# sebproell/4C

Measured on AMD Instinct MI355X. Metric: element-evaluations/sec (hex8 linear elasticity, K+r global assembly), higher is better.
Workload: dtype f64; 1 GPU; hex8-linear-100^3-per-gpu; elements_global=1000000, elements_evaluated_per_gpu=1000000, dofs_owned_rank0=3090903, nnz_rank0=245438109

## Files before the change

4c_amd/csrc/fcg_context.cpp:

```cpp
#include <hip/hip_runtime.h>

#include <algorithm>
#include <chrono>
#include <climits>
#include <cstdlib>
#include <cstring>
#include <mutex>
#include <string>
#include <thread>
#include <vector>

#include "fcg_internal.hpp"
#include "fcg_status.hpp"
#include "fcg_shape.hpp"

namespace {

namespace plan = fcg::create;

std::mutex g_err_mutex;
std::string g_create_error;

void set_create_error(const std::string& s)
{
// ... 214 lines not shown
  U.up<int32_t>(&m.err, nullptr, 3);
  if (U.he == hipSuccess) U.he = hipHostMalloc(reinterpret_cast<void**>(&m.err_host), 2 * sizeof(int32_t),
      hipHostMallocDefault);
}

void upload_structured(Uploader& U, const fcg_desc* d, const plan::NodeRows& N, const plan::StructHost& sp)
{
  fcg::DeviceMesh& m = U.ctx->mesh;
  m.path = FCG_PATH_STRUCTURED;
  m.tiles_x = sp.tiles_x;
  m.tiles_y = sp.tiles_y;
  m.tiles_z = sp.tiles_z;
  m.seg_planes = sp.seg;
  m.I0 = sp.lo[0]; m.J0 = sp.lo[1]; m.K0 = sp.lo[2];
  m.NI = sp.n[0]; m.NJ = sp.n[1]; m.NK = sp.n[2];
  m.EX0 = sp.elo[0]; m.EY0 = sp.elo[1]; m.EZ0 = sp.elo[2];
  m.EX = sp.en[0]; m.EY = sp.en[1]; m.EZ = sp.en[2];
  const char* de = std::getenv("FCG_SWEEP_DEFER");
  m.sweep_defer = de && de[0] ? de[0] == '1'
                              : d->kinematics == FCG_LINEAR && 8 * sp.rows_unordered > N.nrn();
  U.up(&m.elem_at, sp.elem_at);
  U.up(&m.lat_x, sp.lat_x);
  U.up(&m.lat_dof, sp.lat_dof);
  U.up(&m.plane_rec, sp.plane_rec);
  std::vector<double> tab(8 * 8 * 3 * 2 + 8 + 24);
  double xi[81], w[27], xn[81];
  fcg::gauss_rule(fcg::kHex8, xi, w);
  fcg::node_param_coords(fcg::kHex8, xn);
  for (int g = 0; g < 8; ++g) fcg::shape_deriv(fcg::kHex8, &xi[3 * g], &tab[24 * g]);
  for (int g = 0; g < 8; ++g) fcg::shape_deriv(fcg::kHex8, &xn[3 * g], &tab[192 + 24 * g]);
  for (int g = 0; g < 8; ++g) tab[384 + g] = w[g];
  for (int k = 0; k < 24; ++k) tab[392 + k] = xi[k];
  U.up(&m.tables, tab);
}

void upload_colored(Uploader& U, const fcg_desc* d, const plan::Incidences& I, const plan::ColorHost& cp)
{
  fcg::DeviceMesh& m = U.ctx->mesh;
  m.path = FCG_PATH_COLORED;
  U.up(&m.inc_of, I.inc_of);
  U.up(&m.inc_pos, I.inc_pos);
  U.up(&m.inc_row0, I.inc_row0);
  m.h27_pencil = d->material == FCG_MAT_STVK;
  if (m.h27_pencil)
  {
    fcg::upload_h27_tables();
    U.up(&m.col_ele, cp.pen_ele.data(), d->n_ele);
    U.up(&m.pen_ptr, cp.pen_ptr);
    U.up(&m.ele_nb, cp.nb.data(), d->n_ele);
    for (int c = 0; c < 5; ++c) m.pen_color[c] = cp.pen_color[c];
  }
  else
  {
    U.up(&m.col_ele, cp.col_ele.data(), d->n_ele);
    U.up(&m.ele_ft, cp.ft.data(), d->n_ele);
    for (int c = 0; c < 9; ++c) m.color_ptr[c] = cp.color_ptr[c];
  }
}

void upload_gather(Uploader& U, const fcg_desc* d, const plan::GatherHost& G)
{
  fcg::DeviceMesh& m = U.ctx->mesh;
  m.path = FCG_PATH_GATHER;
  m.n_rec = G.n_rec;
  m.n_rec_single = G.n_single;
  m.n_multi = int64_t(G.multi_ptr.size()) - 1;
// ... 479 lines not shown
  }
  return FCG_OK;
}

int fcg_evaluate(fcg_ctx* ctx, int action, const double* u_col, double* fint_row, double* K_vals,
    int32_t* bad_ele_gid)
{
  return fcg_evaluate_host(ctx, action, FCG_ACCUMULATE, u_col, fint_row, K_vals, bad_ele_gid);
}

int fcg_set_timing(fcg_ctx* ctx, int enable)
{
  if (!ctx) return FCG_ERR_ARG;
  ctx->timing.enabled = enable != 0;
  return FCG_OK;
}

int fcg_get_timing(const fcg_ctx* ctx, double* ms_element, double* ms_assemble)
{
  if (!ctx) return FCG_ERR_ARG;
  read_timing(const_cast<fcg_ctx*>(ctx)->timing);
  if (ms_element) *ms_element = ctx->timing.ms_element;
  if (ms_assemble) *ms_assemble = ctx->timing.ms_assemble;
  return 2;
}

int fcg_get_diagnostics(const fcg_ctx* ctx, uint64_t* out, int n)
{
  if (!ctx || !out || n < 0) return FCG_ERR_ARG;
  const fcg::DeviceMesh& m = ctx->mesh;
  unsigned long long v[16] = {};
  if (m.stamps && hipMemcpy(v, m.stamps, sizeof(v), hipMemcpyDeviceToHost) != hipSuccess)
    return fcg_device_error();
  for (int i = 0; i < n && i < 16; ++i) out[i] = v[i];
  return m.stamps ? 16 : 0;
}

int fcg_get_create_phases(const fcg_ctx* ctx, double* out, int n)
{
  if (!ctx || (!out && n > 0)) return FCG_ERR_ARG;
  for (int i = 0; i < n && i < 8; ++i) out[i] = ctx->create_phase_s[i];
  return 8;
}

int fcg_get_info(const fcg_ctx* ctx, fcg_info* info)
{
  if (!ctx || !info) return FCG_ERR_ARG;
  const fcg::DeviceMesh& m = ctx->mesh;
  info->n_ele = m.n_ele;
  info->n_node = m.n_node;
  info->n_rows = m.n_rows;
  info->n_cols = m.n_cols;
  info->nnz = m.nnz;
  info->n_incidences = m.n_inc;
  info->scratch_bytes = !m.scratch ? 0
                                   : (m.h27_nslab > 1 ? m.h27_ring : m.n_inc) *
                                         fcg::record_doubles(m.npe) * int64_t(sizeof(double));
  info->device_bytes = ctx->device_bytes;
  info->path = m.path;
  info->h27_slabs =
      m.path == FCG_PATH_GENERAL && m.h27s ? int32_t(std::max<int64_t>(1, m.h27_nslab)) : 0;
  return FCG_OK;
}

int fcg_set_element_materials(fcg_ctx* ctx, int32_t n_mat, const double* youngs,
    const double* poisson, const int32_t* ele_mat)
// ... 126 lines not shown
```

4c_amd/csrc/fcg_internal.hpp:

```cpp
#pragma once

#include <hip/hip_runtime.h>

#include <cstdint>
#include <string>
#include <vector>

#include "fcg_create_plan.hpp"
#include "fourc_gpu.h"

namespace fcg {

#ifndef FCG_REC27
#define FCG_REC27 256
#endif
constexpr int64_t record_doubles(int npe) { return npe == 27 ? int64_t(FCG_REC27) : 9 * int64_t(npe) + 3; }

struct DeviceMesh {
  int celltype = 0, kinem = 0, npe = 8;
  int64_t n_ele = 0, n_node = 0, n_rows = 0, n_cols = 0, nnz = 0;
  int64_t n_rownodes = 0, n_inc = 0;
  double lambda = 0, mu = 0, cdiag = 0;
  int material = FCG_MAT_STVK;
  double nh_c = 0, nh_beta = 0;
// ... 28 lines not shown
  int64_t* multi_ptr = nullptr;
  int32_t* rec_row0 = nullptr;
  int32_t* rec_meta = nullptr;
  int64_t* rec_base = nullptr;
  int32_t* rec_ele = nullptr;
  uint8_t* rec_a = nullptr;
  uint32_t* rec_tmap = nullptr;
  bool h27s = false;
  int32_t* inc_ele = nullptr;
  uint8_t* inc_a = nullptr;
  int32_t* asm_order = nullptr;
  int32_t* ele_orig = nullptr;
  double* ele_x = nullptr;
  double* ele_gp = nullptr;
  int32_t gp_bad_code = 0, gp_bad_ele = 0;
  int32_t* ele_dof = nullptr;
  double* gather_dummy = nullptr;
  double* apply_ye = nullptr;
  int32_t* apply_dof = nullptr;
  double* diag_de = nullptr;
  uint8_t* diag_dbc = nullptr;
  int64_t h27_nslab = 0, h27_slab = 0, h27_ring = 0;
  int h27_el_grid = 512;
  std::vector<int64_t> h27_asm_ptr;
  int32_t* h27_rows = nullptr;
  int32_t* h27_rslot0 = nullptr;
  int32_t* h27_slot = nullptr;

  int path = FCG_PATH_GENERAL;
  int32_t tiles_x = 0, tiles_y = 0, tiles_z = 0, seg_planes = 0;
  int32_t I0 = 0, J0 = 0, K0 = 0, NI = 0, NJ = 0, NK = 0;
  int32_t EX0 = 0, EY0 = 0, EZ0 = 0, EX = 0, EY = 0, EZ = 0;
  bool sweep_defer = false;
  int32_t* elem_at = nullptr;
  double* lat_x = nullptr;
  int32_t* lat_dof = nullptr;
  uint32_t* plane_rec = nullptr;
  double* tables = nullptr;
  unsigned long long* stamps = nullptr;

  int32_t* col_lid = nullptr;
  int64_t* diag_pos = nullptr;
  bool square_local = false;
  bool owned_cols_first = false;
  bool triple_rows = true;
  double* pcg_work = nullptr;
  int64_t pcg_n = 0;

  int32_t* node_dof_row = nullptr;
  int32_t* node_dof_kcol = nullptr;
  int64_t* mass_ptr = nullptr;
  int64_t* mass_inc = nullptr;
  double* mass_tab = nullptr;
  double* mass_rho = nullptr;
  int32_t* mass_bad = nullptr;
};

hipError_t launch_sweep_h8(const DeviceMesh& m, const double* d_u_col, bool want_k,
    bool overwrite, double* d_K, double* d_fint, hipStream_t stream);

struct SweepTsi {
  const double* v_col = nullptr;
  const double* T_col = nullptr;
  const double* Ngp = nullptr;
  double* Kst = nullptr;
  double* Kts = nullptr;
  double* Ktt = nullptr;
  double* fT = nullptr;
  double m = 0, T0 = 0, conduct = 0, kts = 0;
  bool split = true;
};
hipError_t launch_sweep_h8_tsi(const DeviceMesh& m, const double* d_u_col, bool overwrite,
    double* d_K, double* d_fint, const SweepTsi& t, hipStream_t stream);

struct Timing {
  bool enabled = false;
  bool pending = false;
  int path = 0;
  bool fused = false;
  hipEvent_t ev[3] = {nullptr, nullptr, nullptr};
  double ms_element = 0.0, ms_assemble = 0.0;
};

struct HostStaging {
  double* pin[2] = {nullptr, nullptr};
  hipEvent_t ev[2] = {nullptr, nullptr};
  hipStream_t stream = nullptr;
  int64_t chunk = 0;
  int threads = 8;
};
hipError_t staged_copy(HostStaging& st, int device, void* dst, const void* src, int64_t bytes,
    bool to_device);
// ... 55 lines not shown
```

4c_amd/csrc/fcg_sweep.hip:

```cpp
#include <hip/hip_runtime.h>

#include "fcg_hex8_element.hpp"
#include "fcg_internal.hpp"
#include "fcg_visit_table.h"

namespace fcg {

namespace {

constexpr int TX = 4, TY = 4;
constexpr int EXN = TX + 1, EYN = TY + 1;
constexpr int NSLOT = EXN * EYN;
constexpr int NXN = TX + 2;
constexpr int NNODE = NXN * (TY + 2);
constexpr int PR_ROW0 = 0, PR_LEN = 16, PR_BASE = 32, PR_NPOS = 64;
__device__ constexpr int nx_sw(int p, int slot) { return (p + 4 * (slot & 1)) & 7; }
__device__ constexpr int nx2i(int d, int p, int slot, int n)
{
  return (((d * 4 + p) * NSLOT + slot) * 8 + (n ^ nx_sw(p, slot))) * 2;
}

__device__ constexpr int node_ox(int n) { return ((n & 3) == 1 || (n & 3) == 2) ? 1 : 0; }
__device__ constexpr int node_oy(int n) { return (n & 3) >= 2 ? 1 : 0; }
__device__ constexpr int node_oz(int n) { return n >> 2; }
// ... 48 lines not shown
#ifdef FCG_PROBE_WG3
  double hold[1][9][TSI ? (TH ? 9 : 18) : 9];
#else
#if defined(FCG_HOLD9)
  static constexpr int kHs = 9;
#else
  static constexpr int kHs = 10;
#endif
  alignas(16) double hold[TX * TY + (TSI ? 0 : 1)][9][TSI ? (TH ? 9 : 18) : kHs];
#endif
#ifdef FCG_HOLDLO9
  double hold_lo[DEFER ? TX * TY : 1][9][9];
#else
  alignas(16) double hold_lo[DEFER ? TX * TY : 1][9][10];
#endif
};

__device__ inline int ring(int p) { return (p % 3 + 3) % 3; }

constexpr int kDppXor1 = 0xB1;
constexpr int kDppXor2 = 0x4E;
constexpr int kDppHalfMirror = 0x141;
constexpr int kDppRowRor8 = 0x128;
template <int CTRL>
__device__ inline double dpp_f64(double v)
{
  const int lo = __builtin_amdgcn_mov_dpp(__double2loint(v), CTRL, 0xF, 0xF, false);
  const int hi = __builtin_amdgcn_mov_dpp(__double2hiint(v), CTRL, 0xF, 0xF, false);
  return __hiloint2double(hi, lo);
}

__device__ inline int node_at(int ox, int oy, int oz) { return 4 * oz + (oy ? (ox ? 2 : 3) : (ox ? 1 : 0)); }

template <int KIN, bool TSI, class SH>
__device__ inline void sweep_stage_a(SH& sh, const SweepArgs& A, int s, int g,
    int sx, int sy, int L, int e)
{
  constexpr int NC = node_comps<TSI>();
  const bool valid = e >= 0;
  const double* nd[8];
#pragma unroll
  for (int n = 0; n < 8; ++n)
    nd[n] = sh.node[ring(L + node_oz(n))][(sy + node_oy(n)) * NXN + sx + node_ox(n)];
  const H8dN dn = h8_dn_products(sh.gxi[g][0], sh.gxi[g][1], sh.gxi[g][2]);
  double J[9];
#pragma unroll
  for (int q = 0; q < 9; ++q) J[q] = 0.0;
#pragma unroll
  for (int n = 0; n < 8; ++n)
  {
    const double x0 = nd[n][0], x1 = nd[n][1], x2 = nd[n][2];
    double d0, d1, d2;
    h8_dn(dn, n, d0, d1, d2);
    J[0] += d0 * x0; J[1] += d1 * x0; J[2] += d2 * x0;
    J[3] += d0 * x1; J[4] += d1 * x1; J[5] += d2 * x1;
    J[6] += d0 * x2; J[7] += d1 * x2; J[8] += d2 * x2;
  }
  int bad = 0;
  {
    const int ox = node_ox(g), oy = node_oy(g), oz = node_oz(g);
    const double* zl = sh.node[ring(L)][0];
    const double* zh = sh.node[ring(L + 1)][0];
    const double* pz = oz ? zh : zl;
    const int cxy = (sy + oy) * NXN + sx + ox;
    const double* o = pz + NC * cxy;
    const double* ex_ = pz + NC * (cxy + (ox ? -1 : 1));
    const double* ey_ = pz + NC * (cxy + (oy ? -NXN : NXN));
    const double* ez_ = (oz ? zl : zh) + NC * cxy;
    const double sgx = ox ? 1.0 : -1.0, sgy = oy ? 1.0 : -1.0, sgz = oz ? 1.0 : -1.0;
    const double a0 = sgx * (o[0] - ex_[0]), a1 = sgx * (o[1] - ex_[1]), a2 = sgx * (o[2] - ex_[2]);
    const double b0 = sgy * (o[0] - ey_[0]), b1 = sgy * (o[1] - ey_[1]), b2 = sgy * (o[2] - ey_[2]);
    const double c0 = sgz * (o[0] - ez_[0]), c1 = sgz * (o[1] - ez_[1]), c2 = sgz * (o[2] - ez_[2]);
    const double detn = a0 * (b1 * c2 - b2 * c1) + b0 * (c1 * a2 - c2 * a1) + c0 * (a1 * b2 - a2 * b1);
    if (detn == 0.0) bad = 2;
    else if (!(detn > 0)) bad = 1;
  }
  const double det = h8_invert3x3(J);
  if (det == 0.0) bad = 2;
  else if (TSI && det < 1e-16 && bad == 0) bad = 1;
  const double fac = det * sh.w8[g];
  const double sq = valid ? sqrt(fabs(fac)) : 0.0;
  const double cf = fac < 0.0 ? -sq : sq;
  if (KIN == 0)
  {
#pragma unroll
    for (int q = 0; q < 9; ++q) J[q] *= sq;
  }
  const double ns = KIN == 0 ? 1.0 : sq;
  auto nxyz = [&](int n, double& n0, double& n1, double& n2) {
    double d0, d1, d2;
    h8_dn(dn, n, d0, d1, d2);
    n0 = J[0] * d0 + J[3] * d1 + J[6] * d2;
    n1 = J[1] * d0 + J[4] * d1 + J[7] * d2;
    n2 = J[2] * d0 + J[5] * d1 + J[8] * d2;
  };
  double E[6] = {0, 0, 0, 0, 0, 0};
  double F[9] = {0, 0, 0, 0, 0, 0, 0, 0, 0};
  double Tg = 0.0, trv = 0.0;
#pragma unroll
  for (int n = 0; n < 8; ++n)
  {
    double n0, n1, n2;
    nxyz(n, n0, n1, n2);
    if (TSI)
    {
      trv += n0 * nd[n][6] + n1 * nd[n][7] + n2 * nd[n][8];
      Tg += sh.Ng[TSI ? g : 0][n] * nd[n][9];
    }
    sh.nx[nx2i(0, g >> 1, s, n) + (g & 1)] = KIN == 0 ? n0 : ns * n0;
    sh.nx[nx2i(1, g >> 1, s, n) + (g & 1)] = KIN == 0 ? n1 : ns * n1;
    sh.nx[nx2i(2, g >> 1, s, n) + (g & 1)] = KIN == 0 ? n2 : ns * n2;
    if (KIN == 1)
    {
// ... 17 lines not shown
      for (int q = 0; q < 3; ++q)
        C[r + 3 * q] = F[3 * r] * F[3 * q] + F[3 * r + 1] * F[3 * q + 1] + F[3 * r + 2] * F[3 * q + 2];
    E[0] = 0.5 * (C[0] - 1.0);
    E[1] = 0.5 * (C[4] - 1.0);
    E[2] = 0.5 * (C[8] - 1.0);
    E[3] = C[3];
    E[4] = C[7];
    E[5] = C[2];
  }
  if (KIN == 1)
  {
    const StVK& m = A.mat;
    double S[6];
    S[0] = m.cdiag * E[0] + m.lambda * E[1] + m.lambda * E[2];
    S[1] = m.lambda * E[0] + m.cdiag * E[1] + m.lambda * E[2];
    S[2] = m.lambda * E[0] + m.lambda * E[1] + m.cdiag * E[2];
    S[3] = m.mu * E[3];
    S[4] = m.mu * E[4];
    S[5] = m.mu * E[5];
    double* P = sh.gp[KIN ? g : 0][KIN ? s : 0];
#pragma unroll
    for (int q = 0; q < 9; ++q) P[q] = F[q];
#pragma unroll
    for (int q = 0; q < 6; ++q) P[9 + q] = S[q];
    P[15] = cf;
  }
  if (TSI)
  {
    double* t = sh.tg[TSI ? g : 0][TSI ? s : 0];
    t[0] = cf;
    t[1] = Tg;
    t[2] = A.tsi_m * cf * trv;
  }
  if (valid && bad)
  {
    atomicMax(&A.err[0], bad);
    atomicMin(&A.err[1], e);
  }
  const unsigned long long neg = __ballot(valid && fac < 0.0);
  if (g == 0) sh.neg[s] = uint32_t((neg >> (threadIdx.x & 56)) & 0xFFull);

}

template <int KIN, bool NEG, bool TSI, bool TH = false, class SH>
__device__ inline void sweep_visit(const SH& sh, int slot, int a, int b1, int b2,
    uint32_t nm, double* acc1, double* acc2)
{
#ifndef FCG_TH_PAIRS
#define FCG_TH_PAIRS 1
#endif
  double2 nA[TH && FCG_TH_PAIRS ? 4 : 1], n1[TH && FCG_TH_PAIRS ? 4 : 1], n2[TH && FCG_TH_PAIRS ? 4 : 1];
  if constexpr (TH && FCG_TH_PAIRS)
  {
#pragma unroll
    for (int p = 0; p < 4; ++p)
    {
      nA[p] = *reinterpret_cast<const double2*>(&sh.NgT[a][2 * p]);
      n1[p] = *reinterpret_cast<const double2*>(&sh.NgT[b1][2 * p]);
      n2[p] = *reinterpret_cast<const double2*>(&sh.NgT[b2][2 * p]);
    }
  }
  auto gp_body = [&](int g, double a0, double a1, double a2, double p0, double p1, double p2,
                     double q0, double q1, double q2) {
    if (TH)
    {
      const double* t = sh.tg[g][slot];
#if FCG_TH_PAIRS
      const double2 t01 = *reinterpret_cast<const double2*>(t), t23 = *reinterpret_cast<const double2*>(t + 2);
      const double cf = t01.x, Tg = t01.y, qq = t23.x;
      const double Na = (g & 1) ? nA[g >> 1].y : nA[g >> 1].x, N1 = (g & 1) ? n1[g >> 1].y : n1[g >> 1].x,
                   N2 = (g & 1) ? n2[g >> 1].y : n2[g >> 1].x;
#else
      const double cf = t[0], Tg = t[1], qq = t[2];
      const double Na = sh.Ng[g][a], N1 = sh.Ng[g][b1], N2 = sh.Ng[g][b2];
// ... 136 lines not shown
__device__ inline void block_k(const StVK& m, const double* acc, double* Kb)
{
  const double lam = m.lambda, mu = m.mu;
#pragma unroll
  for (int r = 0; r < 3; ++r)
#pragma unroll
    for (int q = 0; q < 3; ++q) Kb[3 * r + q] = lam * acc[3 * r + q] + mu * acc[3 * q + r];
  if (KIN == 0)
  {
    const double tr = mu * (acc[0] + acc[4] + acc[8]);
    Kb[0] += tr;
    Kb[4] += tr;
    Kb[8] += tr;
  }
  else
  {
    Kb[0] += mu * acc[9] + acc[15];
    Kb[4] += mu * acc[10] + acc[15];
    Kb[8] += mu * acc[11] + acc[15];
    Kb[1] += mu * acc[12]; Kb[3] += mu * acc[12];
    Kb[5] += mu * acc[13]; Kb[7] += mu * acc[13];
    Kb[2] += mu * acc[14]; Kb[6] += mu * acc[14];
  }
}

#define FCG_STAMP(i)                                                                               \
  if (A.stamps && tid == 0)                                                                        \
  {                                                                                                \
    const unsigned long long now = __builtin_amdgcn_s_memtime();                                  \
    st_acc[i] += now - st_last;                                                                    \
    st_last = now;                                                                                 \
  }

template <int KIN, bool WANT_K, bool OVERWRITE, int MODE>
#ifndef FCG_SWEEP_WGS
#define FCG_SWEEP_WGS 2
#endif
__global__ __launch_bounds__(256, KIN ? 1 : FCG_SWEEP_WGS) void sweep_h8_kernel(SweepArgs A)
{
  constexpr bool TSI = MODE == 1 || MODE == 2, TH = MODE == 2, DEFER = MODE == 3;
  static_assert(!TSI || (KIN == 0 && WANT_K), "TSI is geometrically linear, full tangent");
  static_assert(!DEFER || WANT_K, "deferred blocks are K blocks");
  __shared__ SweepShared<KIN, TSI, TH, DEFER> sh;
  constexpr int NACC = TH ? 8 : ((KIN || TSI) ? 16 : 9);
  constexpr int NC = node_comps<TSI>();
  constexpr int NLD = (NNODE * NC + 255) / 256;
  constexpr int NF = TSI ? 4 : 3;
  const int tid = threadIdx.x;
  unsigned long long st_acc[3] = {0, 0, 0};
  unsigned long long st_last = A.stamps ? __builtin_amdgcn_s_memtime() : 0ull;
  const int tile = blockIdx.x;
  const int tx = tile % A.tiles_x;
  const int ty = (tile / A.tiles_x) % A.tiles_y;
  const int tz = tile / (A.tiles_x * A.tiles_y);
  const int i0 = A.I0 + TX * tx, j0 = A.J0 + TY * ty;
  const int kz0 = A.K0 + A.seg_planes * tz;
  const int kz1 = min(kz0 + A.seg_planes, A.K0 + A.NK);
  const uint32_t* prec_tile = A.plane_rec + (int64_t(ty) * A.tiles_x + tx) * A.NK * PLANE_REC_WORDS;
  const int64_t LX = A.EX + 1, LY = A.EY + 1;

  if (tid < 24) sh.gxi[tid / 3][tid % 3] = A.tables[392 + tid];
  if (tid < 8) sh.w8[tid] = A.tables[384 + tid];
  if (TSI && tid < 64)
  {
    (&sh.Ng[0][0])[tid] = A.Ngp[tid];
    sh.NgT[TSI ? (tid & 7) : 0][tid >> 3] = A.Ngp[tid];
  }

  const int s = tid >> 3, g = tid & 7;
  const bool a_lane = s < NSLOT;
  const int sx = s % EXN, sy = s / EXN;
  const int ex = i0 - 1 + sx, ey = j0 - 1 + sy;
  const bool exy_in = a_lane && ex >= A.EX0 && ex < A.EX0 + A.EX && ey >= A.EY0 && ey < A.EY0 + A.EY;
  auto load_elem = [&](int lz) -> int {
    if (!exy_in || lz < A.EZ0 || lz >= A.EZ0 + A.EZ) return -1;
    return A.elem_at[(int64_t(lz - A.EZ0) * A.EY + (ey - A.EY0)) * A.EX + (ex - A.EX0)];
  };
  bool n_lane[NLD], nxy_in[NLD];
  int ncol[NLD], ncomp[NLD];
  int64_t nlat_xy[NLD];
#pragma unroll
  for (int j = 0; j < NLD; ++j)
  {
    const int v = tid + 256 * j;
    n_lane[j] = v < NNODE * NC;
    ncol[j] = v / NC;
    ncomp[j] = v - NC * (v / NC);
    const int ni = i0 - 1 + ncol[j] % NXN, nj = j0 - 1 + ncol[j] / NXN;
    nxy_in[j] = n_lane[j] && ni >= A.EX0 && ni <= A.EX0 + A.EX && nj >= A.EY0 && nj <= A.EY0 + A.EY;
    nlat_xy[j] = nxy_in[j] ? int64_t(nj - A.EY0) * LX + (ni - A.EX0) : 0;
  }
  auto node_li = [&](int j, int P) -> int64_t { return int64_t(P - A.EZ0) * LX * LY + nlat_xy[j]; };
  auto node_in = [&](int j, int P) -> bool { return nxy_in[j] && P >= A.EZ0 && P <= A.EZ0 + A.EZ; };
  auto load_dof = [&](int j, int P) -> int32_t {
    if (!node_in(j, P) || ncomp[j] < 3) return -1;
    return A.lat_dof[node_li(j, P)];
  };
  auto load_val = [&](int j, int P, int32_t dof) -> double {
    if (!node_in(j, P)) return 0.0;
    const int cp = ncomp[j];
    if (cp < 3) return A.lat_x[3 * node_li(j, P) + cp];
    if (dof < 0) return 0.0;
    if (!TSI || cp < 6) return A.u_col[dof + cp - 3];
    if (cp < 9) return A.v_col[dof + cp - 6];
    return A.T_col[dof / 3];
  };
  auto load_node = [&](int j, int P) -> double { return load_val(j, P, load_dof(j, P)); };
  auto load_rec = [&](int p, uint32_t* w) {
    const bool in = p >= kz0 && p < kz1;
    const uint32_t* src = prec_tile + int64_t(in ? p - A.K0 : 0) * PLANE_REC_WORDS;
#pragma unroll
    for (int k = 0; k < 2; ++k)
    {
      const int v = tid + 256 * k;
      if (v < PLANE_REC_WORDS) w[k] = in ? src[v] : (v < PR_LEN ? 0xFFFFFFFFu : 0u);
    }
  };
  auto store_rec = [&](int p, const uint32_t* w) {
#pragma unroll
    for (int k = 0; k < 2; ++k)
    {
      const int v = tid + 256 * k;
      if (v < PLANE_REC_WORDS) sh.prec[ring(p)][v] = w[k];
    }
  };

  const int c = tid >> 4, k = tid & 15;
  const int cx = c % TX, cy = c / TX;
  const uint32_t vis0 = kVisit[k][0], vis1 = kVisit[k][1];

#pragma unroll
  for (int j = 0; j < NLD; ++j)
    if (n_lane[j])
    {
      sh.node[ring(kz0 - 1)][ncol[j]][ncomp[j]] = load_node(j, kz0 - 1);
      sh.node[ring(kz0)][ncol[j]][ncomp[j]] = load_node(j, kz0);
    }
  {
// ... 6 lines not shown
  int32_t dof_nxt[NLD];
#pragma unroll
  for (int j = 0; j < NLD; ++j) dof_nxt[j] = n_lane[j] ? load_dof(j, kz0 + 1) : -1;
  int e_cur = load_elem(kz0 - 1);
  for (int v = tid; v < int(sizeof(sh.hold) / sizeof(double)); v += 256) (&sh.hold[0][0][0])[v] = 0.0;
  double fkeep[NF];
#pragma unroll
  for (int d = 0; d < NF; ++d) fkeep[d] = 0.0;
  __builtin_amdgcn_s_waitcnt(0);
  __syncthreads();

  for (int L = kz0 - 1; L < kz1; ++L)
  {
    const int e_nxt = load_elem(L + 1);
    double node_nxt[NLD];
    int32_t dof_nn[NLD];
#pragma unroll
    for (int j = 0; j < NLD; ++j)
    {
#ifdef FCG_PROBE_TH_NOPREFETCH
      if (TH)
      {
        node_nxt[j] = 0.0;
        dof_nn[j] = -1;
        continue;
      }
#endif
      node_nxt[j] = n_lane[j] ? load_val(j, L + 2, dof_nxt[j]) : 0.0;
      dof_nn[j] = n_lane[j] ? load_dof(j, L + 3) : -1;
    }
    uint32_t rec_nxt[2];
    load_rec(L + 2, rec_nxt);
#ifdef FCG_PROBE_NOSTAGEA
    if (a_lane && e_cur == -12345) sweep_stage_a<KIN, TSI>(sh, A, s, g, sx, sy, L, e_cur);
#else
    if (a_lane) sweep_stage_a<KIN, TSI>(sh, A, s, g, sx, sy, L, e_cur);
#endif
    __syncthreads();
    FCG_STAMP(0);
#pragma unroll
    for (int j = 0; j < NLD; ++j)
    {
      if (n_lane[j]) sh.node[ring(L + 2)][ncol[j]][ncomp[j]] = node_nxt[j];
      dof_nxt[j] = dof_nn[j];
    }
    store_rec(L + 2, rec_nxt);
#ifdef FCG_SWEEP_COMMIT_STAMP
    if (A.stamps)
    {
      __asm__ volatile("" ::"v"(rec_nxt[0]), "v"(node_nxt[0]));
      FCG_STAMP(2);
    }
#endif

    const bool wl = L >= kz0, wl1 = L + 1 < kz1;
    constexpr bool kRingSel = !TSI && !DEFER;
    const int rL = ring(L), rL1 = ring(L + 1);
    const uint32_t* recL = sh.prec[rL];
    const uint32_t* recL1 = sh.prec[rL1];
    double fpart[NF];
#pragma unroll
    for (int d = 0; d < NF; ++d) fpart[d] = 0.0;
    if (WANT_K || KIN == 0)
    {
#ifdef FCG_PROBE_WG3
      constexpr bool kProbeWg3 = true;
#else
      constexpr bool kProbeWg3 = false;
#endif
      constexpr bool kBranchFree = !TSI && !DEFER && !kProbeWg3;
      struct EmitIn {
        int32_t row0, len32;
        uint32_t base_lo, base_hi;
        uint16_t pos;
        const double* ub;
        double u0, u1, u2;
        double* h;
        double held[9];
      };
// ... 188 lines not shown
            if (OVERWRITE)
              d2[r] = Tv[3 + r];
            else
              d2[r] += Tv[3 + r];
          }
#pragma unroll
          for (int r = 0; r < 3; ++r)
          {
            double* d1 = A.Kst + bst + r * lst + pst;
            if (OVERWRITE)
              *d1 = Tv[r];
            else
              *d1 += Tv[r];
          }
          }
          double* d3 = A.Ktt + base / 9 + pst;
          if (OVERWRITE)
            *d3 = Tv[6];
          else
            *d3 += Tv[6];
        }
      };
      auto emit = [&](int act, int t, double* Kb, double* Tv) {
        EmitIn in;
        emit_load(act, t, in);
        __asm__ volatile("" ::: "memory");
        emit_finish(act, t, in, Kb, Tv);
      };
      double acc1[NACC], acc2[NACC];
#pragma unroll
      for (int i = 0; i < NACC; ++i) acc1[i] = acc2[i] = 0.0;
      auto slot_of = [&](uint32_t w) { return (cx + int(w & 1)) + EXN * (cy + int((w >> 1) & 1)); };
      uint32_t nm_pre[2] = {0u, 0u};
      if constexpr (!TSI)
      {
        nm_pre[0] = sh.neg[slot_of(vis0)];
        nm_pre[1] = sh.neg[slot_of(vis1)];
      }
#ifndef FCG_SWEEP_VISIT_UNROLL
#define FCG_SWEEP_VISIT_UNROLL (!TSI && KIN == 0)
#endif
      constexpr int kVisitUnroll = (FCG_SWEEP_VISIT_UNROLL) ? 2 : 1;
      constexpr bool kPairEmits = kVisitUnroll == 2 && kBranchFree;
      double Kb2[9];
#pragma unroll kVisitUnroll
      for (int v = 0; v < 2; ++v)
      {
        const uint32_t w = v == 0 ? vis0 : vis1;
        const int a = (w >> 2) & 7, b1 = (w >> 5) & 7, b2 = (w >> 8) & 7;
        const int slot = slot_of(w);
        const uint32_t nm = TSI ? sh.neg[slot] : (v == 0 ? nm_pre[0] : nm_pre[1]);
        if (nm == 0u)
          sweep_visit<KIN, false, TSI, TH>(sh, slot, a, b1, b2, nm, acc1, acc2);
        else
          sweep_visit<KIN, true, TSI, TH>(sh, slot, a, b1, b2, nm, acc1, acc2);
        if ((w >> 24) & 1u)
        {
          double Kb[9], Tv[7];
          if (!TH) block_k<KIN>(A.mat, acc2, Kb);
          if (TSI) tsi_block<TH>(A, acc2, Tv);
#pragma unroll
          for (int i = 0; i < NACC; ++i) acc2[i] = 0.0;
          if (kPairEmits && v == 1)
          {
#pragma unroll
            for (int i = 0; i < 9; ++i) Kb2[i] = Kb[i];
          }
          else
            emit(int((w >> 21) & 7), int((w >> 16) & 31), Kb, Tv);
        }
      }
      {
        const int pair = int((vis1 >> 26) & 3);
        double Kb[9], Tv[7];
        if (!TH)
        {
          block_k<KIN>(A.mat, acc1, Kb);
#pragma unroll
          for (int i = 0; i < 9; ++i)
          {
            const double o = dpp_f64<kDppXor1>(Kb[i]);
            Kb[i] = pair == kPairRecv ? Kb[i] + o : Kb[i];
          }
        }
        if (TSI)
        {
          tsi_block<TH>(A, acc1, Tv);
#pragma unroll
// ... 100 lines not shown
  if (A.stamps && tid == 0)
  {
    for (int i = 0; i < 3; ++i) atomicAdd(&A.stamps[i], st_acc[i]);
    atomicAdd(&A.stamps[5], 1ull);
  }
}

}

namespace {
SweepArgs sweep_args(const DeviceMesh& m, const double* d_u_col, double* d_K, double* d_fint)
{
  SweepArgs a{};
  a.u_col = d_u_col;
  a.lat_x = m.lat_x;
  a.lat_dof = m.lat_dof;
  a.elem_at = m.elem_at;
  a.plane_rec = m.plane_rec;
  a.tables = m.tables;
  a.K = d_K;
  a.fint = d_fint;
  a.err = m.err;
  a.stamps = m.stamps;
  a.mat = StVK{m.lambda, m.mu, m.cdiag};
  a.tiles_x = m.tiles_x;
  a.tiles_y = m.tiles_y;
  a.seg_planes = m.seg_planes;
  a.I0 = m.I0; a.J0 = m.J0; a.K0 = m.K0; a.NI = m.NI; a.NJ = m.NJ; a.NK = m.NK;
  a.EX0 = m.EX0; a.EY0 = m.EY0; a.EZ0 = m.EZ0; a.EX = m.EX; a.EY = m.EY; a.EZ = m.EZ;
  return a;
}
}

#define FCG_SWEEP(KIN)                                                                             \
  if (want_k && m.sweep_defer && overwrite)                                                        \
    hipLaunchKernelGGL((sweep_h8_kernel<KIN, true, true, 3>), grid, block, 0, stream, a);      \
  else if (want_k && m.sweep_defer)                                                                \
    hipLaunchKernelGGL((sweep_h8_kernel<KIN, true, false, 3>), grid, block, 0, stream, a);     \
  else if (want_k && overwrite)                                                                    \
    hipLaunchKernelGGL((sweep_h8_kernel<KIN, true, true, 0>), grid, block, 0, stream, a);      \
  else if (want_k)                                                                                 \
    hipLaunchKernelGGL((sweep_h8_kernel<KIN, true, false, 0>), grid, block, 0, stream, a);     \
  else if (overwrite)                                                                              \
    hipLaunchKernelGGL((sweep_h8_kernel<KIN, false, true, 0>), grid, block, 0, stream, a);     \
  else                                                                                             \
    hipLaunchKernelGGL((sweep_h8_kernel<KIN, false, false, 0>), grid, block, 0, stream, a);

hipError_t launch_sweep_h8_totlag(const DeviceMesh& m, const double* d_u_col, bool want_k,
    bool overwrite, double* d_K, double* d_fint, hipStream_t stream);

#ifdef FCG_SWEEP_TOTLAG_TU
hipError_t launch_sweep_h8_totlag(const DeviceMesh& m, const double* d_u_col, bool want_k,
    bool overwrite, double* d_K, double* d_fint, hipStream_t stream)
{
  const int64_t ntiles = int64_t(m.tiles_x) * m.tiles_y * m.tiles_z;
  if (ntiles == 0) return hipSuccess;
  const SweepArgs a = sweep_args(m, d_u_col, d_K, d_fint);
  const dim3 grid{static_cast<unsigned>(ntiles), 1, 1};
  const dim3 block{256, 1, 1};
  FCG_SWEEP(1)
  return hipGetLastError();
}
#else
hipError_t launch_sweep_h8(const DeviceMesh& m, const double* d_u_col, bool want_k,
    bool overwrite, double* d_K, double* d_fint, hipStream_t stream)
{
  if (m.kinem != 0) return launch_sweep_h8_totlag(m, d_u_col, want_k, overwrite, d_K, d_fint, stream);
  const int64_t ntiles = int64_t(m.tiles_x) * m.tiles_y * m.tiles_z;
  if (ntiles == 0) return hipSuccess;
  const SweepArgs a = sweep_args(m, d_u_col, d_K, d_fint);
  const dim3 grid{static_cast<unsigned>(ntiles), 1, 1};
  const dim3 block{256, 1, 1};
  FCG_SWEEP(0)
  return hipGetLastError();
}

hipError_t launch_sweep_h8_tsi(const DeviceMesh& m, const double* d_u_col, bool overwrite,
    double* d_K, double* d_fint, const SweepTsi& t, hipStream_t stream)
{
  const int64_t ntiles = int64_t(m.tiles_x) * m.tiles_y * m.tiles_z;
  if (ntiles == 0) return hipSuccess;
  SweepArgs a = sweep_args(m, d_u_col, d_K, d_fint);
  a.v_col = t.v_col;
  a.T_col = t.T_col;
  a.Ngp = t.Ngp;
  a.Kst = t.Kst;
  a.Kts = t.Kts;
  a.Ktt = t.Ktt;
  a.fT = t.fT;
  a.tsi_m = t.m;
  a.tsi_T0 = t.T0;
  a.tsi_k = t.conduct;
  a.tsi_kts = t.kts;
  const dim3 grid{static_cast<unsigned>(ntiles), 1, 1};
  const dim3 block{256, 1, 1};
  if (!t.split)
  {
    if (overwrite)
      hipLaunchKernelGGL((sweep_h8_kernel<0, true, true, 1>), grid, block, 0, stream, a);
    else
      hipLaunchKernelGGL((sweep_h8_kernel<0, true, false, 1>), grid, block, 0, stream, a);
    return hipGetLastError();
  }
  if (overwrite)
  {
    hipLaunchKernelGGL((sweep_h8_kernel<0, true, true, 0>), grid, block, 0, stream, a);
    hipLaunchKernelGGL((sweep_h8_kernel<0, true, true, 2>), grid, block, 0, stream, a);
  }
  else
  {
    hipLaunchKernelGGL((sweep_h8_kernel<0, true, false, 0>), grid, block, 0, stream, a);
    hipLaunchKernelGGL((sweep_h8_kernel<0, true, false, 2>), grid, block, 0, stream, a);
  }
  return hipGetLastError();
}
#endif
#undef FCG_SWEEP

}
```

4c_amd/fcg.py:

```python

import ctypes
import os

import numpy as np

PKG_DIR = os.path.dirname(os.path.abspath(__file__))
LIB_PATH = os.path.join(PKG_DIR, "lib", "libfourc_gpu.so")
if os.environ.get("FCG_LIB"):
    LIB_PATH = os.path.join(PKG_DIR, "lib", "libfourc_gpu_%s.so" % os.environ["FCG_LIB"])

HEX8, HEX27 = 0, 1
LINEAR, TOTLAG = 0, 1
CALC_NLNSTIFF, CALC_INTERNALFORCE = 0, 1
ACCUMULATE, OVERWRITE = 0, 1
PATH_AUTO, PATH_GENERAL, PATH_STRUCTURED, PATH_COLORED, PATH_GATHER = 0, 1, 2, 3, 4
MAT_STVK, MAT_ELASTHYPER_COUPNEOHOOKE = 0, 1
TSI_STRUCT_FORCE, TSI_STIFFTEMP, TSI_THERMO_FINTCOND, TSI_COUPLTANG = 1, 2, 4, 8
TSI_ALL = 15
ABI_VERSION = 2

FCG_OK, FCG_ERR_NODAL_DETJ, FCG_ERR_SINGULAR, FCG_ERR_ARG, FCG_ERR_DEVICE = 0, 1, 2, 3, 4
STATUS = {0: "FCG_OK", 1: "FCG_ERR_NODAL_DETJ", 2: "FCG_ERR_SINGULAR", 3: "FCG_ERR_ARG",
          4: "FCG_ERR_DEVICE"}

# ... 759 lines not shown
        rc = lib().fcg_mass_assemble(self._h, float(density), rp, int(mode), _tensor_ptr(out),
                                     self._stream(stream))
        if rc != 0:
            self._raise(rc, -1)
        lib().fcg_get_info(self._h, ctypes.byref(self.info))
        return out

    def mass_nodal(self, density, ele_density=None, m_node=None, m_lumped=None, stream=None):
        if m_node is None and m_lumped is None:
            m_node, m_lumped = self._f64(self.info.nnz // 9), self._f64(self.info.n_rows)
        rho, rp = self._ele_density(ele_density)
        rc = lib().fcg_mass_nodal(self._h, float(density), rp, _tensor_ptr(m_node),
                                  _tensor_ptr(m_lumped), self._stream(stream))
        if rc != 0:
            self._raise(rc, -1)
        lib().fcg_get_info(self._h, ctypes.byref(self.info))
        return m_node, m_lumped

    def effective_tangent(self, cK, cM, m_node, K_vals=None, x_col=None, y_row=None, stream=None):
        rc = lib().fcg_effective_tangent(self._h, float(cK), float(cM), _tensor_ptr(m_node),
                                         _tensor_ptr(K_vals), _tensor_ptr(x_col), _tensor_ptr(y_row),
                                         self._stream(stream))
        if rc != 0:
            self._raise(rc, -1)

    def set_timing(self, enable):
        lib().fcg_set_timing(self._h, 1 if enable else 0)

    def diagnostics(self):
        buf = (ctypes.c_uint64 * 16)()
        n = lib().fcg_get_diagnostics(self._h, buf, 16)
        return list(buf) if n > 0 else None

    CREATE_PHASES = ("checks", "graph_device", "node_rows", "lattice_plans", "incidences",
                     "incidence_positions", "device_plans", "total")

    def create_phases(self):
        buf = (ctypes.c_double * 8)()
        lib().fcg_get_create_phases(self._h, buf, 8)
        return dict(zip(self.CREATE_PHASES, list(buf)))

    def timing(self):
        a, b = ctypes.c_double(), ctypes.c_double()
        lib().fcg_get_timing(self._h, ctypes.byref(a), ctypes.byref(b))
        return a.value, b.value


class TsiGraph:

    def __init__(self, mesh):
        nn = mesh.n_node
        self.node_dof_col_t = np.ascontiguousarray(mesh.node_dof_col // 3, dtype=np.int32)
        self.node_dof_row_t = np.ascontiguousarray(
            np.where(mesh.node_dof_row >= 0, mesh.node_dof_row // 3, -1), dtype=np.int32)
        self.n_rows_t = int(mesh.n_rows) // 3
        self.n_cols_t = int(mesh.n_cols) // 3
        assert len(self.node_dof_col_t) == nn
        rp = np.asarray(mesh.rowptr, dtype=np.int64)
        cl = np.asarray(mesh.col_lid)
        starts = rp[0:-1:3]
        nnb = (rp[1::3] - rp[0:-1:3]) // 3
        tot = int(nnb.sum())
        self.rowptr_tt = np.concatenate([[0], np.cumsum(nnb)]).astype(np.int64)
        off = np.arange(tot, dtype=np.int64) - np.repeat(self.rowptr_tt[:-1], nnb)
        self.col_tt = np.ascontiguousarray(cl[np.repeat(starts, nnb) + 3 * off] // 3, dtype=np.int32)
        n3 = np.repeat(nnb, 3)
# ... 112 lines not shown
```

include/fourc_gpu.h:

```cpp
#ifndef FOURC_GPU_H
#define FOURC_GPU_H

#include <stdint.h>

#ifdef __cplusplus
extern "C" {
#endif

#define FCG_ABI_VERSION 2

enum fcg_celltype { FCG_HEX8 = 0, FCG_HEX27 = 1 };
enum fcg_kinem { FCG_LINEAR = 0, FCG_TOTLAG = 1 };
enum fcg_action { FCG_CALC_NLNSTIFF = 0, FCG_CALC_INTERNALFORCE = 1 };
enum fcg_mode { FCG_ACCUMULATE = 0, FCG_OVERWRITE = 1 };

enum fcg_status {
  FCG_OK = 0,
  FCG_ERR_NODAL_DETJ = 1,
  FCG_ERR_SINGULAR = 2,
  FCG_ERR_ARG = 3,
  FCG_ERR_DEVICE = 4
};

typedef struct fcg_desc {
// ... 37 lines not shown
int fcg_evaluate(fcg_ctx* ctx, int action, const double* u_col, double* fint_row, double* K_vals,
    int32_t* bad_ele_gid);

int fcg_evaluate_device(fcg_ctx* ctx, int action, int mode, const double* d_u_col,
    double* d_fint_row, double* d_K_vals, void* stream, int32_t* bad_ele_gid);

int fcg_device_alloc(int device, int64_t bytes, void** d_ptr);
int fcg_device_free(void* d_ptr);
int fcg_memcpy_h2d(void* d_dst, const void* h_src, int64_t bytes);
int fcg_memcpy_d2h(void* h_dst, const void* d_src, int64_t bytes);
int fcg_memset_device(void* d_dst, int value, int64_t bytes);

int fcg_set_timing(fcg_ctx* ctx, int enable);
int fcg_get_timing(const fcg_ctx* ctx, double* ms_element, double* ms_assemble);

typedef struct fcg_info {
  int64_t n_ele, n_node, n_rows, n_cols, nnz;
  int64_t n_incidences;
  int64_t scratch_bytes;
  int64_t device_bytes;
  int32_t path;
  int32_t h27_slabs;
} fcg_info;
int fcg_get_info(const fcg_ctx* ctx, fcg_info* info);

int fcg_get_graph(const fcg_ctx* ctx, int64_t* rowptr, int32_t* col_lid, int64_t col_capacity,
    int64_t* nnz);

int fcg_measure_peaks(int device, double* hbm_triad_gbs, double* fp64_valu_tflops,
    double* fp64_mfma_tflops);

int fcg_measure_hbm(int device, double* copy_gbs, double* write_gbs);

int fcg_get_diagnostics(const fcg_ctx* ctx, uint64_t* out, int n);

int fcg_get_create_phases(const fcg_ctx* ctx, double* out, int n);

int fcg_spmv(fcg_ctx* ctx, const double* d_K_vals, const double* d_x_col, double* d_y_row,
    void* stream);
int fcg_dirichlet_apply(fcg_ctx* ctx, int64_t n_dbc, const int32_t* d_rows, double* d_K_vals,
    double* d_rhs_row, double* d_freact_row, void* stream);
int fcg_mass_assemble(fcg_ctx* ctx, double density, const double* ele_density ,
    int mode , double* d_M_vals , void* stream);
int fcg_mass_nodal(fcg_ctx* ctx, double density, const double* ele_density,
    double* d_m_node , double* d_m_lumped_row , void* stream);
int fcg_effective_tangent(fcg_ctx* ctx, double cK, double cM, const double* d_m_node,
    double* d_K_vals , const double* d_x_col, double* d_y_row ,
    void* stream);
int fcg_spmv_f32(fcg_ctx* ctx, const float* d_K32, const double* d_x_col, double* d_y_row,
    void* stream);
int fcg_tangent_apply(fcg_ctx* ctx, const double* d_u_col, const double* d_x_col, double* d_y_row,
    void* stream);
int fcg_pcg_solve(fcg_ctx* ctx, const double* d_K_vals, const double* d_b_row, double* d_x_row,
    double rtol, int max_iter, int* iterations, double* rel_residual, void* stream);
int fcg_block_jacobi_setup(fcg_ctx* ctx, const double* d_K_vals, double* d_dinv, void* stream);
int fcg_block_jacobi_apply(fcg_ctx* ctx, const double* d_dinv, const double* d_r_row, double* d_z_row,
    double scale, int accumulate, void* stream);
int fcg_tangent_diag(fcg_ctx* ctx, const double* d_u_col, int64_t n_dbc, const int32_t* d_dbc_rows,
    double* d_diag, double* d_dinv, void* stream);
int fcg_chebyshev_step(fcg_ctx* ctx, const double* d_dinv, const double* d_b_row, const double* d_y_row,
    double* d_d_row, double* d_x_row, double c_d, double c_r, int mode, void* stream);
int fcg_node_transfer(int device, int64_t n_out, const int64_t* d_ptr, const int32_t* d_src_row0,
    const double* d_w, const int32_t* d_dst_row0, const double* d_x, double* d_y, int accumulate,
    void* stream);
int fcg_box_stencil_apply(int device, int nx, int ny, int nz, const int32_t* d_row_of,
    const uint8_t* d_clamped, const double* d_S, const double* d_x, double* d_y, void* stream);
// ... 240 lines not shown
```

Before: 1.102 billion element-evaluations/s.

## Validate reference geometry once at setup and dispatch an unchecked sweep kernel

A one-time geometry pass at context creation runs a stripped-down instantiation of the structured hex8 sweep kernel. It records invalid Jacobians and negative determinants in the reference configuration. If none are found, evaluation launches a CHECKED=false kernel that skips per-Gauss-point nodal determinant checks, the negative-det ballot and shared-memory mask, and the negative-weight visit branch. It also makes node value loads branch-free and adds a scheduling barrier. The cost is extra template instantiations and a setup-time kernel plus sync, and totlag paths may lose checks that depend on the current configuration.

```diff
diff --git a/4c_amd/csrc/fcg_context.cpp b/4c_amd/csrc/fcg_context.cpp
--- a/4c_amd/csrc/fcg_context.cpp
+++ b/4c_amd/csrc/fcg_context.cpp
@@ -270,6 +270,8 @@
   for (int g = 0; g < 8; ++g) tab[384 + g] = w[g];
   for (int k = 0; k < 24; ++k) tab[392 + k] = xi[k];
   U.up(&m.tables, tab);
+  const char* ck = std::getenv("FCG_SWEEP_CHECKED");
+  if (U.he == hipSuccess) U.chk(fcg::sweep_geometry_pass(m, ck && ck[0] == '1', U.ctx->stream));
 }
 
 void upload_colored(Uploader& U, const fcg_desc* d, const plan::Incidences& I, const plan::ColorHost& cp)
@@ -815,6 +817,8 @@
   unsigned long long v[16] = {};
   if (m.stamps && hipMemcpy(v, m.stamps, sizeof(v), hipMemcpyDeviceToHost) != hipSuccess)
     return fcg_device_error();
+  v[15] = m.path != FCG_PATH_STRUCTURED ? FCG_SWEEP_KERNEL_NA
+                                        : (m.sweep_checked ? FCG_SWEEP_KERNEL_CHECKED : FCG_SWEEP_KERNEL_UNCHECKED);
   for (int i = 0; i < n && i < 16; ++i) out[i] = v[i];
   return m.stamps ? 16 : 0;
 }
diff --git a/4c_amd/csrc/fcg_internal.hpp b/4c_amd/csrc/fcg_internal.hpp
--- a/4c_amd/csrc/fcg_internal.hpp
+++ b/4c_amd/csrc/fcg_internal.hpp
@@ -84,6 +84,8 @@
   int32_t I0 = 0, J0 = 0, K0 = 0, NI = 0, NJ = 0, NK = 0;
   int32_t EX0 = 0, EY0 = 0, EZ0 = 0, EX = 0, EY = 0, EZ = 0;
   bool sweep_defer = false;
+  int32_t geom_code = 0, geom_ele = INT32_MAX;
+  bool geom_neg = false, sweep_checked = true;
   int32_t* elem_at = nullptr;
   double* lat_x = nullptr;
   int32_t* lat_dof = nullptr;
@@ -110,6 +112,8 @@
 
 hipError_t launch_sweep_h8(const DeviceMesh& m, const double* d_u_col, bool want_k,
     bool overwrite, double* d_K, double* d_fint, hipStream_t stream);
+
+hipError_t sweep_geometry_pass(DeviceMesh& m, bool force_checked, hipStream_t stream);
 
 struct SweepTsi {
   const double* v_col = nullptr;
diff --git a/4c_amd/csrc/fcg_sweep.hip b/4c_amd/csrc/fcg_sweep.hip
--- a/4c_amd/csrc/fcg_sweep.hip
+++ b/4c_amd/csrc/fcg_sweep.hip
@@ -104,7 +104,7 @@
 
 __device__ inline int node_at(int ox, int oy, int oz) { return 4 * oz + (oy ? (ox ? 2 : 3) : (ox ? 1 : 0)); }
 
-template <int KIN, bool TSI, class SH>
+template <int KIN, bool TSI, bool CHECKED, bool GEOM, class SH>
 __device__ inline void sweep_stage_a(SH& sh, const SweepArgs& A, int s, int g,
     int sx, int sy, int L, int e)
 {
@@ -114,14 +114,21 @@
 #pragma unroll
   for (int n = 0; n < 8; ++n)
     nd[n] = sh.node[ring(L + node_oz(n))][(sy + node_oy(n)) * NXN + sx + node_ox(n)];
-  const H8dN dn = h8_dn_products(sh.gxi[g][0], sh.gxi[g][1], sh.gxi[g][2]);
+  double X[8][3];
+#pragma unroll
+  for (int n = 0; n < 8; ++n)
+#pragma unroll
+    for (int d = 0; d < 3; ++d) X[n][d] = nd[n][d];
+  const double gx0 = sh.gxi[g][0], gx1 = sh.gxi[g][1], gx2 = sh.gxi[g][2], wg = sh.w8[g];
+  if constexpr (!CHECKED) __builtin_amdgcn_sched_barrier(0);
+  const H8dN dn = h8_dn_products(gx0, gx1, gx2);
   double J[9];
 #pragma unroll
   for (int q = 0; q < 9; ++q) J[q] = 0.0;
 #pragma unroll
   for (int n = 0; n < 8; ++n)
   {
-    const double x0 = nd[n][0], x1 = nd[n][1], x2 = nd[n][2];
+    const double x0 = X[n][0], x1 = X[n][1], x2 = X[n][2];
     double d0, d1, d2;
     h8_dn(dn, n, d0, d1, d2);
     J[0] += d0 * x0; J[1] += d1 * x0; J[2] += d2 * x0;
@@ -129,6 +136,7 @@
     J[6] += d0 * x2; J[7] += d1 * x2; J[8] += d2 * x2;
   }
   int bad = 0;
+  if constexpr (CHECKED)
   {
     const int ox = node_ox(g), oy = node_oy(g), oz = node_oz(g);
     const double* zl = sh.node[ring(L)][0];
@@ -148,9 +156,19 @@
     else if (!(detn > 0)) bad = 1;
   }
   const double det = h8_invert3x3(J);
-  if (det == 0.0) bad = 2;
+  if (CHECKED && det == 0.0) bad = 2;
   else if (TSI && det < 1e-16 && bad == 0) bad = 1;
-  const double fac = det * sh.w8[g];
+  const double fac = det * wg;
+  if constexpr (GEOM)
+  {
+    if (valid && bad)
+    {
+      atomicMax(&A.err[0], bad);
+      atomicMin(&A.err[1], e);
+    }
+    if (valid && fac < 0.0) atomicMax(&A.err[2], 1);
+    return;
+  }
   const double sq = valid ? sqrt(fabs(fac)) : 0.0;
   const double cf = fac < 0.0 ? -sq : sq;
   if (KIN == 0)
@@ -234,14 +252,19 @@
     t[1] = Tg;
     t[2] = A.tsi_m * cf * trv;
   }
-  if (valid && bad)
-  {
-    atomicMax(&A.err[0], bad);
-    atomicMin(&A.err[1], e);
-  }
-  const unsigned long long neg = __ballot(valid && fac < 0.0);
-  if (g == 0) sh.neg[s] = uint32_t((neg >> (threadIdx.x & 56)) & 0xFFull);
-
+  if constexpr (CHECKED || KIN == 1)
+  {
+    if (valid && bad)
+    {
+      atomicMax(&A.err[0], bad);
+      atomicMin(&A.err[1], e);
+    }
+  }
+  if constexpr (CHECKED)
+  {
+    const unsigned long long neg = __ballot(valid && fac < 0.0);
+    if (g == 0) sh.neg[s] = uint32_t((neg >> (threadIdx.x & 56)) & 0xFFull);
+  }
 }
 
 template <int KIN, bool NEG, bool TSI, bool TH = false, class SH>
@@ -444,13 +467,15 @@
     st_last = now;                                                                                 \
   }
 
-template <int KIN, bool WANT_K, bool OVERWRITE, int MODE>
+template <int KIN, bool WANT_K, bool OVERWRITE, int MODE, bool CHECKED = true>
 #ifndef FCG_SWEEP_WGS
 #define FCG_SWEEP_WGS 2
 #endif
 __global__ __launch_bounds__(256, KIN ? 1 : FCG_SWEEP_WGS) void sweep_h8_kernel(SweepArgs A)
 {
-  constexpr bool TSI = MODE == 1 || MODE == 2, TH = MODE == 2, DEFER = MODE == 3;
+  constexpr bool TSI = MODE == 1 || MODE == 2, TH = MODE == 2, DEFER = MODE == 3, GEOM = MODE == 4;
+  static_assert(!GEOM || (KIN == 0 && !WANT_K && CHECKED), "the geometry pass is one instantiation");
+  static_assert(CHECKED || !TSI, "the TSI passes keep the checks");
   static_assert(!TSI || (KIN == 0 && WANT_K), "TSI is geometrically linear, full tangent");
   static_assert(!DEFER || WANT_K, "deferred blocks are K blocks");
   __shared__ SweepShared<KIN, TSI, TH, DEFER> sh;
@@ -505,17 +530,17 @@
   auto node_li = [&](int j, int P) -> int64_t { return int64_t(P - A.EZ0) * LX * LY + nlat_xy[j]; };
   auto node_in = [&](int j, int P) -> bool { return nxy_in[j] && P >= A.EZ0 && P <= A.EZ0 + A.EZ; };
   auto load_dof = [&](int j, int P) -> int32_t {
-    if (!node_in(j, P) || ncomp[j] < 3) return -1;
+    if (GEOM || !node_in(j, P) || ncomp[j] < 3) return -1;
     return A.lat_dof[node_li(j, P)];
   };
   auto load_val = [&](int j, int P, int32_t dof) -> double {
-    if (!node_in(j, P)) return 0.0;
     const int cp = ncomp[j];
-    if (cp < 3) return A.lat_x[3 * node_li(j, P) + cp];
-    if (dof < 0) return 0.0;
-    if (!TSI || cp < 6) return A.u_col[dof + cp - 3];
-    if (cp < 9) return A.v_col[dof + cp - 6];
-    return A.T_col[dof / 3];
+    const bool has = node_in(j, P) && (cp < 3 || dof >= 0);
+    const double* src = A.lat_x + (3 * node_li(j, P) + cp);
+    if (cp >= 3) src = A.u_col + (dof + cp - 3);
+    if (TSI && cp >= 6) src = A.v_col + (dof + cp - 6);
+    if (TSI && cp >= 9) src = A.T_col + dof / 3;
+    return has ? *src : 0.0;
   };
   auto load_node = [&](int j, int P) -> double { return load_val(j, P, load_dof(j, P)); };
   auto load_rec = [&](int p, uint32_t* w) {
@@ -588,9 +613,9 @@
     uint32_t rec_nxt[2];
     load_rec(L + 2, rec_nxt);
 #ifdef FCG_PROBE_NOSTAGEA
-    if (a_lane && e_cur == -12345) sweep_stage_a<KIN, TSI>(sh, A, s, g, sx, sy, L, e_cur);
-#else
-    if (a_lane) sweep_stage_a<KIN, TSI>(sh, A, s, g, sx, sy, L, e_cur);
+    if (a_lane && e_cur == -12345) sweep_stage_a<KIN, TSI, CHECKED, GEOM>(sh, A, s, g, sx, sy, L, e_cur);
+#else
+    if (a_lane) sweep_stage_a<KIN, TSI, CHECKED, GEOM>(sh, A, s, g, sx, sy, L, e_cur);
 #endif
     __syncthreads();
     FCG_STAMP(0);
@@ -601,6 +626,12 @@
       dof_nxt[j] = dof_nn[j];
     }
     store_rec(L + 2, rec_nxt);
+    if constexpr (GEOM)
+    {
+      e_cur = e_nxt;
+      __syncthreads();
+      continue;
+    }
 #ifdef FCG_SWEEP_COMMIT_STAMP
     if (A.stamps)
     {
@@ -855,7 +886,7 @@
       for (int i = 0; i < NACC; ++i) acc1[i] = acc2[i] = 0.0;
       auto slot_of = [&](uint32_t w) { return (cx + int(w & 1)) + EXN * (cy + int((w >> 1) & 1)); };
       uint32_t nm_pre[2] = {0u, 0u};
-      if constexpr (!TSI)
+      if constexpr (!TSI && CHECKED)
       {
         nm_pre[0] = sh.neg[slot_of(vis0)];
         nm_pre[1] = sh.neg[slot_of(vis1)];
@@ -872,11 +903,20 @@
         const uint32_t w = v == 0 ? vis0 : vis1;
         const int a = (w >> 2) & 7, b1 = (w >> 5) & 7, b2 = (w >> 8) & 7;
         const int slot = slot_of(w);
-        const uint32_t nm = TSI ? sh.neg[slot] : (v == 0 ? nm_pre[0] : nm_pre[1]);
-        if (nm == 0u)
-          sweep_visit<KIN, false, TSI, TH>(sh, slot, a, b1, b2, nm, acc1, acc2);
+        if constexpr (!CHECKED)
+        {
+          uint32_t always = 0u;
+          __asm__ volatile("" : "+s"(always));
+          if (always == 0u) sweep_visit<KIN, false, TSI, TH>(sh, slot, a, b1, b2, 0u, acc1, acc2);
+        }
         else
-          sweep_visit<KIN, true, TSI, TH>(sh, slot, a, b1, b2, nm, acc1, acc2);
+        {
+          const uint32_t nm = TSI ? sh.neg[slot] : (v == 0 ? nm_pre[0] : nm_pre[1]);
+          if (nm == 0u)
+            sweep_visit<KIN, false, TSI, TH>(sh, slot, a, b1, b2, nm, acc1, acc2);
+          else
+            sweep_visit<KIN, true, TSI, TH>(sh, slot, a, b1, b2, nm, acc1, acc2);
+        }
         if ((w >> 24) & 1u)
         {
           double Kb[9], Tv[7];
@@ -1043,19 +1083,28 @@
 }
 }
 
+#define FCG_SWEEP_C(KIN, CHECKED)                                                                  \
+  if (want_k && m.sweep_defer && overwrite)                                                        \
+    hipLaunchKernelGGL((sweep_h8_kernel<KIN, true, true, 3, CHECKED>), grid, block, 0, stream, a);  \
+  else if (want_k && m.sweep_defer)                                                                \
+    hipLaunchKernelGGL((sweep_h8_kernel<KIN, true, false, 3, CHECKED>), grid, block, 0, stream, a); \
+  else if (want_k && overwrite)                                                                    \
+    hipLaunchKernelGGL((sweep_h8_kernel<KIN, true, true, 0, CHECKED>), grid, block, 0, stream, a);  \
+  else if (want_k)                                                                                 \
+    hipLaunchKernelGGL((sweep_h8_kernel<KIN, true, false, 0, CHECKED>), grid, block, 0, stream, a); \
+  else if (overwrite)                                                                              \
+    hipLaunchKernelGGL((sweep_h8_kernel<KIN, false, true, 0, CHECKED>), grid, block, 0, stream, a); \
+  else                                                                                             \
+    hipLaunchKernelGGL((sweep_h8_kernel<KIN, false, false, 0, CHECKED>), grid, block, 0, stream, a);
 #define FCG_SWEEP(KIN)                                                                             \
-  if (want_k && m.sweep_defer && overwrite)                                                        \
-    hipLaunchKernelGGL((sweep_h8_kernel<KIN, true, true, 3>), grid, block, 0, stream, a);      \
-  else if (want_k && m.sweep_defer)                                                                \
-    hipLaunchKernelGGL((sweep_h8_kernel<KIN, true, false, 3>), grid, block, 0, stream, a);     \
-  else if (want_k && overwrite)                                                                    \
-    hipLaunchKernelGGL((sweep_h8_kernel<KIN, true, true, 0>), grid, block, 0, stream, a);      \
-  else if (want_k)                                                                                 \
-    hipLaunchKernelGGL((sweep_h8_kernel<KIN, true, false, 0>), grid, block, 0, stream, a);     \
-  else if (overwrite)                                                                              \
-    hipLaunchKernelGGL((sweep_h8_kernel<KIN, false, true, 0>), grid, block, 0, stream, a);     \
+  if (m.sweep_checked)                                                                             \
+  {                                                                                                \
+    FCG_SWEEP_C(KIN, true)                                                                         \
+  }                                                                                                \
   else                                                                                             \
-    hipLaunchKernelGGL((sweep_h8_kernel<KIN, false, false, 0>), grid, block, 0, stream, a);
+  {                                                                                                \
+    FCG_SWEEP_C(KIN, false)                                                                        \
+  }
 
 hipError_t launch_sweep_h8_totlag(const DeviceMesh& m, const double* d_u_col, bool want_k,
     bool overwrite, double* d_K, double* d_fint, hipStream_t stream);
@@ -1084,6 +1133,42 @@
   const dim3 block{256, 1, 1};
   FCG_SWEEP(0)
   return hipGetLastError();
+}
+
+hipError_t sweep_geometry_pass(DeviceMesh& m, bool force_checked, hipStream_t stream)
+{
+  m.geom_code = 0;
+  m.geom_ele = INT32_MAX;
+  m.geom_neg = false;
+  m.sweep_checked = true;
+  const int64_t ntiles = int64_t(m.tiles_x) * m.tiles_y * m.tiles_z;
+  if (ntiles > 0)
+  {
+    int32_t* d_out = nullptr;
+    int32_t out[3] = {0, INT32_MAX, 0};
+    hipError_t he = hipMalloc(reinterpret_cast<void**>(&d_out), sizeof(out));
+    if (he != hipSuccess) return he;
+    he = hipMemcpyAsync(d_out, out, sizeof(out), hipMemcpyHostToDevice, stream);
+    if (he == hipSuccess)
+    {
+      SweepArgs a = sweep_args(m, nullptr, nullptr, nullptr);
+      a.err = d_out;
+      a.stamps = nullptr;
+      const dim3 grid{static_cast<unsigned>(ntiles), 1, 1};
+      const dim3 block{256, 1, 1};
+      hipLaunchKernelGGL((sweep_h8_kernel<0, false, false, 4>), grid, block, 0, stream, a);
+      he = hipGetLastError();
+    }
+    if (he == hipSuccess) he = hipMemcpyAsync(out, d_out, sizeof(out), hipMemcpyDeviceToHost, stream);
+    if (he == hipSuccess) he = hipStreamSynchronize(stream);
+    (void)hipFree(d_out);
+    if (he != hipSuccess) return he;
+    m.geom_code = out[0];
+    m.geom_ele = out[1];
+    m.geom_neg = out[2] != 0;
+  }
+  m.sweep_checked = force_checked || m.geom_code != 0 || m.geom_neg;
+  return hipSuccess;
 }
 
 hipError_t launch_sweep_h8_tsi(const DeviceMesh& m, const double* d_u_col, bool overwrite,
@@ -1127,5 +1212,6 @@
 }
 #endif
 #undef FCG_SWEEP
-
-}
+#undef FCG_SWEEP_C
+
+}
diff --git a/4c_amd/fcg.py b/4c_amd/fcg.py
--- a/4c_amd/fcg.py
+++ b/4c_amd/fcg.py
@@ -815,6 +815,13 @@
         n = lib().fcg_get_diagnostics(self._h, buf, 16)
         return list(buf) if n > 0 else None
 
+    SWEEP_KERNELS = ("not applicable", "checked", "unchecked")
+
+    def sweep_kernel(self):
+        buf = (ctypes.c_uint64 * 16)()
+        lib().fcg_get_diagnostics(self._h, buf, 16)
+        return self.SWEEP_KERNELS[int(buf[15])]
+
     CREATE_PHASES = ("checks", "graph_device", "node_rows", "lattice_plans", "incidences",
                      "incidence_positions", "device_plans", "total")
 
diff --git a/include/fourc_gpu.h b/include/fourc_gpu.h
--- a/include/fourc_gpu.h
+++ b/include/fourc_gpu.h
@@ -93,6 +93,9 @@
 
 int fcg_measure_hbm(int device, double* copy_gbs, double* write_gbs);
 
+#define FCG_SWEEP_KERNEL_NA 0
+#define FCG_SWEEP_KERNEL_CHECKED 1
+#define FCG_SWEEP_KERNEL_UNCHECKED 2
 int fcg_get_diagnostics(const fcg_ctx* ctx, uint64_t* out, int n);
 
 int fcg_get_create_phases(const fcg_ctx* ctx, double* out, int n);
```

New measurement: 1.147 billion element-evaluations/s (median of 6 runs). +4.0%, better.
